# pashtari/factorizer

Measured on AMD Instinct MI355X. Metric: volumes/sec fwd+bwd, Swin Factorizer 128^3, higher is better.
Workload: dtype f32

## Files before the change

### factorizer_amd/csrc/nmf_cf.h

```cpp
#pragma once
#include <cstdlib>

#include "fz_common.h"
#include "nmf_core.h"
#include "nmf_gram.h"

namespace fz {

struct CfGeom {
  int B, C, D, H, W;
  int h;
  int G0, G1, G2;
  int s0, s1, s2;
  int accumulate;
  int divisor;
  float gscale_div;
  int64_t plane;
  int ps0, ps1, ps2;
};

enum { CF_PLAIN = 0, CF_STORE_FACTORS = 1, CF_FROM_FACTORS = 2 };
constexpr int CFG_COFAC = 88;

struct CfWave {
  using F = float;
  int lane;
  __device__ __forceinline__ int col(int j) const {
    const int jp = j >> 2, e = j & 3;
    return (((jp * 4 + (lane >> 4)) * 8 + ((lane >> 1) & 7)) * 8) + (lane & 1) * 4 + e;
  }
  __device__ __forceinline__ float sum(float v) const { return wave_sum(v); }
  __device__ __forceinline__ void sum8(float (&v)[8]) const { wave_sum8(v, lane); }
  __device__ __forceinline__ void st_priv(float* base, int idx, float v) const { base[idx * 64 + lane] = v; }
  __device__ __forceinline__ float ld_priv(const float* base, int idx) const { return base[idx * 64 + lane]; }
  __device__ __forceinline__ void st_uni(float* base, int idx, float v) const {
    if (lane == 0) base[idx] = v;
  }
  __device__ __forceinline__ float ld_uni(const float* base, int idx) const { return base[idx]; }
  __device__ __forceinline__ float ld_uni_global(const float* p, int idx) const { return p[idx]; }
  __device__ __forceinline__ float ld_v0(const float* v0, int j, int r, int R) const { return v0[col(j) * R + r]; }
  __device__ __forceinline__ float keep_col(int, float v) const { return v; }
  __device__ __forceinline__ void fence() const { __builtin_amdgcn_fence(__ATOMIC_ACQ_REL, "wavefront"); }
  static constexpr bool kDistRows = true;
  __device__ __forceinline__ float sum8_dist(const float (&v)[8]) const { return wave_sum8_dist(v, lane); }
  __device__ __forceinline__ float grp_take(float d, int m) const {
    return __int_as_float(__builtin_amdgcn_readlane(__float_as_int(d), 8 * m));
  }
  __device__ __forceinline__ bool grp_below(int n) const { return (lane >> 3) < n; }
  __device__ __forceinline__ void st_grp(float* base, int i0, int stride, float d) const {
    if ((lane & 7) == 0) base[i0 + (lane >> 3) * stride] = d;
  }
  __device__ __forceinline__ float ld_grp_global(const float* p, int i0, int stride) const { return p[i0 + (lane >> 3) * stride]; }
  __device__ __forceinline__ float ld_grp(const float* base, int i0, int stride) const { return base[i0 + (lane >> 3) * stride]; }
  __device__ __forceinline__ float grp_sum(float d) const { return wave_group_sum(d); }
  __device__ __forceinline__ float mask_rows(float d, int mreal) const { return (lane >> 3) < mreal ? d : 0.f; }
  __device__ __forceinline__ float pick_call(int c, float tot, float mine) const { return (lane & 7) == c ? tot : mine; }
  __device__ __forceinline__ void k_unrotate(float* scratch, float mine, float (&Kd)[8]) const {
    const int g = lane >> 3;
    scratch[g * 8 + ((g + lane) & 7)] = mine;
    fence();
    const float4 a = *reinterpret_cast<const float4*>(scratch + g * 8), b = *reinterpret_cast<const float4*>(scratch + g * 8 + 4);
    Kd[0] = a.x; Kd[1] = a.y; Kd[2] = a.z; Kd[3] = a.w; Kd[4] = b.x; Kd[5] = b.y; Kd[6] = b.z; Kd[7] = b.w;
    fence();
  }
};

struct CfAddr {
  int64_t base;
  int64_t off[2];
  int64_t V;
};

__device__ __forceinline__ void cf_decode(const CfGeom& q, int64_t mat, int lane, CfAddr& a) {
  unsigned t = (unsigned)mat;
  const int g2 = (int)(t % (unsigned)q.G2); t /= (unsigned)q.G2;
  const int g1 = (int)(t % (unsigned)q.G1); t /= (unsigned)q.G1;
  const int g0 = (int)(t % (unsigned)q.G0); t /= (unsigned)q.G0;
  const int hh = (int)(t % (unsigned)q.h);
  const int b = (int)(t / (unsigned)q.h);
  const int p1 = (lane >> 1) & 7, half = lane & 1;
  int z1 = g1 * 8 + p1 - q.s1; if (z1 < 0) z1 += q.H;
  int z2 = g2 * 8 + half * 4 - q.s2; if (z2 < 0) z2 += q.W;
  a.V = q.plane;
  a.base = ((int64_t)b * q.C + (int64_t)hh * 8) * a.V;
#pragma unroll
  for (int jp = 0; jp < 2; ++jp) {
    int z0 = g0 * 8 + jp * 4 + (lane >> 4) - q.s0; if (z0 < 0) z0 += q.D;
    a.off[jp] = ((int64_t)z0 * q.H + z1) * q.W + z2;
  }
}

template <typename AT>
__device__ __forceinline__ void cf_load(const AT* __restrict__ t, const CfAddr& a, float (&x)[8][8]) {
#pragma unroll
  for (int dd = 0; dd < 8; ++dd)
#pragma unroll
    for (int jp = 0; jp < 2; ++jp) {
      const float4 v = ld4(t + a.base + dd * a.V + a.off[jp]);
      x[dd][jp * 4 + 0] = v.x; x[dd][jp * 4 + 1] = v.y; x[dd][jp * 4 + 2] = v.z; x[dd][jp * 4 + 3] = v.w;
    }
}

__device__ __forceinline__ bool cf_pow2(float dv) { return (__float_as_uint(dv) & 0x007fffffu) == 0u && dv > 0.f; }

__device__ __forceinline__ void cf_divide(float (&g)[8][8], float dv) {
  if (dv == 1.0f) return;
  if (cf_pow2(dv)) {
    const float inv = 1.0f / dv;
#pragma unroll
    for (int dd = 0; dd < 8; ++dd)
#pragma unroll
      for (int j = 0; j < 8; ++j) g[dd][j] = g[dd][j] * inv;
  } else {
#pragma unroll
    for (int dd = 0; dd < 8; ++dd)
#pragma unroll
      for (int j = 0; j < 8; ++j) g[dd][j] = g[dd][j] / dv;
  }
}

__device__ __forceinline__ float4 cf_divide4(float4 o, float dv, bool pow2) {
  if (pow2) {
    const float inv = 1.0f / dv;
    o.x *= inv; o.y *= inv; o.z *= inv; o.w *= inv;
  } else {
    o.x /= dv; o.y /= dv; o.z /= dv; o.w /= dv;
  }
  return o;
}

__device__ __forceinline__ int64_t cf_logical_block(int xcd_remap) {
  const int64_t nb = gridDim.x;
  const int64_t bid = (xcd_remap & 2) ? nb - 1 - (int64_t)blockIdx.x : (int64_t)blockIdx.x;
  if (!(xcd_remap & 1) || nb < 16) return bid;
  const int64_t q = nb / 8, r = nb % 8, xcd = bid % 8, i = bid / 8;
  return (xcd < r ? xcd * (q + 1) : r * (q + 1) + (xcd - r) * q) + i;
}

template <int WPB>
struct CfTile {
  static constexpr bool SWZ = WPB == 8 || WPB == 4;
  static constexpr int LW = SWZ ? WPB * 8 : WPB * 8 + 8;
  static constexpr int NT = WPB * 64;
  static constexpr int CHUNKS = WPB * 2;
  static constexpr int STAGE_FLOATS = 2 * 64 * LW;
  static __device__ __forceinline__ int at(int row, int chunk) {
    if (WPB == 8) return row * LW + ((chunk ^ (2 * (row & 7))) << 2);
    if (WPB == 4) return row * LW + ((chunk ^ (2 * (((row >> 1) & 1) | ((((row & 1) ^ (row >> 2)) & 1) << 1)))) << 2);
    return row * LW + chunk * 4;
  }
};

template <typename AT>
__device__ __forceinline__ const AT* cf_at(const AT* p, unsigned o) {
  return reinterpret_cast<const AT*>(reinterpret_cast<const char*>(p) + o * (unsigned)sizeof(AT));
}
template <typename AT>
__device__ __forceinline__ AT* cf_at(AT* p, unsigned o) {
  return reinterpret_cast<AT*>(reinterpret_cast<char*>(p) + o * (unsigned)sizeof(AT));
}
template <bool HALF, typename AT>
__device__ __forceinline__ float4 cf_ld4(const AT* p, unsigned o, unsigned o2) {
  if (HALF) {
    float a[2], b[2];
    aload<2>(cf_at(p, o), a);
    aload<2>(cf_at(p, o2), b);
    return make_float4(a[0], a[1], b[0], b[1]);
  }
  return ld4(cf_at(p, o));
}
template <bool HALF, typename AT>
__device__ __forceinline__ void cf_st4(AT* p, unsigned o, unsigned o2, float4 v) {
  if (HALF) {
    const float a[2] = {v.x, v.y}, b[2] = {v.z, v.w};
    astore<2>(cf_at(p, o), a);
// ... 121 lines not shown
```

### factorizer_amd/csrc/nmf_cf.hip

```cpp
#include "nmf_cf.h"

namespace fz {

static void cf_norm_shift(const int* shift, int D, int H, int W, int (&s)[3]) {
  const int S[3] = {D, H, W};
  for (int i = 0; i < 3; ++i) { s[i] = shift[i] % S[i]; if (s[i] < 0) s[i] += S[i]; }
}

static int cf_geom(CfGeom& q, int B, int C, int D, int H, int W, const int* shift, const int* prev_shift, int accumulate,
                   int divisor) {
  if (B < 0 || C < 8 || (C % 8) || D < 8 || H < 8 || W < 8 || (D % 8) || (H % 8) || (W % 8))
    return fail(FZ_E_SHAPE, "fz_nmf_cf: needs C % 8 == 0 and spatial dims multiples of 8");
  if (!shift) return fail(FZ_E_ARG, "fz_nmf_cf: shift is null");
  if ((int64_t)D * H * W >= ((int64_t)1 << 30)) return fail(FZ_E_UNSUPPORTED, "fz_nmf_cf: 2^30 or more voxels per channel plane");
  q.B = B; q.C = C; q.D = D; q.H = H; q.W = W; q.h = C / 8; q.G0 = D / 8; q.G1 = H / 8; q.G2 = W / 8;
  int s[3], ps[3] = {0, 0, 0};
  cf_norm_shift(shift, D, H, W, s);
  if (s[2] % 2) return fail(FZ_E_UNSUPPORTED, "fz_nmf_cf: W-axis shift must be even");
  if (prev_shift) cf_norm_shift(prev_shift, D, H, W, ps);
  q.s0 = s[0]; q.s1 = s[1]; q.s2 = s[2];
  q.ps0 = ps[0]; q.ps1 = ps[1]; q.ps2 = ps[2];
  q.accumulate = accumulate; q.divisor = divisor; q.gscale_div = 1.0f;
  q.plane = (int64_t)D * H * W;
#ifdef FZ_PROBE_PLANE_PAD
  q.plane += FZ_PROBE_PLANE_PAD;
#endif
  return FZ_OK;
}

template <class Checks>
static int cf_prepare(CfLaunch& a, int B, int C, int D, int H, int W, const int* shift, const int* prev_shift, int accumulate,
                      int divisor, fz_stream_t stream, Checks checks) {
  int rc = cf_geom(a.q, B, C, D, H, W, shift, prev_shift, accumulate, divisor);
  if (rc == FZ_OK) rc = checks(a.q);
  if (rc != FZ_OK) return rc;
  a.nmat = (int64_t)B * a.q.h * a.q.G0 * a.q.G1 * a.q.G2;
  if (a.nmat >= (int64_t)1 << 31) return fail(FZ_E_UNSUPPORTED, "fz_nmf_cf: more than 2^31 matrices");
  a.xr = 1 | (tile_order() << 1);
  a.st = (hipStream_t)stream;
  return FZ_OK;
}

template <class F>
static int cf_with_dtype(int act_dtype, const char* bad, F f) {
  if (act_dtype == FZ_STORE_F32) return f(float{});
  if (act_dtype == FZ_STORE_BF16) return f(bf16{});
  return fail(FZ_E_ARG, bad);
}

}

using namespace fz;

extern "C" int fz_nmf_cf_supported(int C, int D, int H, int W, int d, int pd, int ph, int pw, int R, int T, int Tgrad) {
  if (d != 8 || pd != 8 || ph != 8 || pw != 8 || (C % 8) || (D % 8) || (H % 8) || (W % 8)) return 0;
  if (R < 1 || R > 2 || T < 0 || (int64_t)D * H * W >= ((int64_t)1 << 30)) return 0;
  const int G = Tgrad < 0 ? 0 : (Tgrad > T ? T : Tgrad);
  const int per_wave = (R == 1 ? Hist<8, 8, 1>::floats(G) : Hist<8, 8, 2>::floats(G)) * (int)sizeof(float);
  return per_wave <= 160 * 1024 ? 1 : 0;
}

extern "C" int fz_nmf_cf_fwd(const void* t, const float* u0, const float* v0, void* out, int B, int C, int D,
                             int H, int W, const int* shift, int accumulate, int divisor, int R, int T,
                             int solver, float eps, int act_dtype, fz_stream_t stream) {
  return cf_with_dtype(act_dtype, "fz_nmf_cf_fwd: bad act_dtype", [&](auto at) {
    using AT = decltype(at);
    CfLaunch a;
    const int rc = cf_prepare(a, B, C, D, H, W, shift, nullptr, accumulate, divisor, stream, [&](const CfGeom&) {
      if (!t || !u0 || !v0 || !out) return fail(FZ_E_ARG, "fz_nmf_cf_fwd: null pointer");
      if (R < 1 || R > 2) return fail(FZ_E_UNSUPPORTED, "fz_nmf_cf_fwd: rank 1..2");
      if (solver < FZ_SOLVER_MU || solver > FZ_SOLVER_SMU) return fail(FZ_E_ARG, "fz_nmf_cf_fwd: bad solver");
      return (int)FZ_OK;
    });
    if (rc != FZ_OK || a.nmat == 0) return rc;
    return cf_fwd_launch<AT>((const AT*)t, u0, v0, (AT*)out, nullptr, nullptr, a, CF_PLAIN, R, T, solver, eps);
  });
}

extern "C" int fz_nmf_cf_bwd(const void* t, const float* u0, const float* v0, const void* ga, void* gt, int B,
                             int C, int D, int H, int W, const int* shift, int accumulate, int nshift,
                             int relu_gate, int R, int T, int Tgrad, int solver, float eps, int act_dtype,
                             fz_stream_t stream) {
  return cf_with_dtype(act_dtype, "fz_nmf_cf_bwd: bad act_dtype", [&](auto at) {
    using AT = decltype(at);
    CfLaunch a;
    const int rc = cf_prepare(a, B, C, D, H, W, shift, nullptr, accumulate, 1, stream, [&](const CfGeom&) {
      if (!t || !u0 || !v0 || !ga || !gt) return fail(FZ_E_ARG, "fz_nmf_cf_bwd: null pointer");
      if (R < 1 || R > 2) return fail(FZ_E_UNSUPPORTED, "fz_nmf_cf_bwd: rank 1..2");
      if (solver < FZ_SOLVER_MU || solver > FZ_SOLVER_SMU) return fail(FZ_E_ARG, "fz_nmf_cf_bwd: bad solver");
      return (int)FZ_OK;
    });
    if (rc != FZ_OK || a.nmat == 0) return rc;
    a.q.gscale_div = (float)(nshift > 1 ? nshift : 1);
    const int G = Tgrad < 0 ? 0 : (Tgrad > T ? T : Tgrad);
    return cf_bwd_launch<AT>((const AT*)t, u0, v0, (const AT*)ga, (AT*)gt, a, relu_gate, R, T, G, solver, eps);
  });
}

extern "C" int fz_nmf_cf_factors_supported(int C, int D, int H, int W, int d, int pd, int ph, int pw, int R, int T, int Tgrad,
                                           int nshift, const int* shifts) {
  if (!fz_nmf_cf_supported(C, D, H, W, d, pd, ph, pw, R, T, Tgrad)) return 0;
  if (R != 1 || nshift != 2 || !shifts || (W % 64)) return 0;
  for (int w = 0; w < 2; ++w) {
    int s[3];
    cf_norm_shift(shifts + 3 * w, D, H, W, s);
    if (s[2] % 4) return 0;
  }
  return 1;
}

static int cf_fwd_factors(const void* t, const float* u0, const float* v0, void* out, float* vfac, float* ufac, int B, int C,
                          int D, int H, int W, const int* shift, const int* prev_shift, int form, int divisor, int R, int T,
                          int solver, float eps, int act_dtype, fz_stream_t stream, const char* null_msg, const char* dtype_msg) {
  return cf_with_dtype(act_dtype, dtype_msg, [&](auto at) {
    using AT = decltype(at);
    CfLaunch a;
    const int rc = cf_prepare(a, B, C, D, H, W, shift, prev_shift, form == CF_FROM_FACTORS, divisor, stream, [&](const CfGeom& q) {
      if (!t || !u0 || !v0 || !vfac || !ufac || (form == CF_FROM_FACTORS && (!out || !prev_shift))) return fail(FZ_E_ARG, null_msg);
      if (R != 1) return fail(FZ_E_UNSUPPORTED, "fz_nmf_cf_fwd factor forms: rank 1 only");
      if (W % 64) return fail(FZ_E_UNSUPPORTED, "fz_nmf_cf_fwd factor forms: W must be a multiple of 64");
      if (solver < FZ_SOLVER_MU || solver > FZ_SOLVER_SMU) return fail(FZ_E_ARG, "fz_nmf_cf_fwd factor forms: bad solver");
      if (divisor < 1) return fail(FZ_E_ARG, "fz_nmf_cf_fwd factor forms: divisor < 1");
      if ((q.s2 % 4) || (q.ps2 % 4)) return fail(FZ_E_UNSUPPORTED, "fz_nmf_cf_fwd factor forms: W-axis shift must be a multiple of 4");
      return (int)FZ_OK;
    });
    if (rc != FZ_OK || a.nmat == 0) return rc;
    return cf_fwd_launch<AT>((const AT*)t, u0, v0, (AT*)out, vfac, ufac, a, form, R, T, solver, eps);
  });
}

extern "C" int fz_nmf_cf_fwd_store_factors(const void* t, const float* u0, const float* v0, float* vfac, float* ufac, int B,
                                           int C, int D, int H, int W, const int* shift, int R, int T, int solver, float eps,
                                           int act_dtype, fz_stream_t stream) {
  return cf_fwd_factors(t, u0, v0, nullptr, vfac, ufac, B, C, D, H, W, shift, nullptr, CF_STORE_FACTORS, 1, R, T, solver, eps,
                        act_dtype, stream, "fz_nmf_cf_fwd_store_factors: null pointer (t, u0, v0, vfac or ufac)",
                        "fz_nmf_cf_fwd_store_factors: bad act_dtype");
}

extern "C" int fz_nmf_cf_fwd_from_factors(const void* t, const float* u0, const float* v0, const float* vfac,
                                          const float* ufac, void* out, int B, int C, int D, int H, int W, const int* shift,
                                          const int* prev_shift, int divisor, int R, int T, int solver, float eps, int act_dtype,
                                          fz_stream_t stream) {
  return cf_fwd_factors(t, u0, v0, out, const_cast<float*>(vfac), const_cast<float*>(ufac), B, C, D, H, W, shift, prev_shift,
                        CF_FROM_FACTORS, divisor, R, T, solver, eps, act_dtype, stream,
                        "fz_nmf_cf_fwd_from_factors: null pointer (t, u0, v0, vfac, ufac, out or prev_shift)",
                        "fz_nmf_cf_fwd_from_factors: bad act_dtype");
}

extern "C" int fz_nmf_cf_bwd_factors_supported(int C, int D, int H, int W, int d, int pd, int ph, int pw, int R, int T, int Tgrad,
                                               int solver, int relu_gate, int nshift, const int* shifts) {
  if (FZ_KNOB("FZ_CF_BWD_FACTORS").set && FZ_KNOB("FZ_CF_BWD_FACTORS").val == 0) return 0;
  if (!fz_nmf_cf_factors_supported(C, D, H, W, d, pd, ph, pw, R, T, Tgrad, nshift, shifts)) return 0;
  if (solver != FZ_SOLVER_HALS || !relu_gate) return 0;
  if (T < 1 || Tgrad < T) return 0;
  if ((C / 8) * (int64_t)(D / 8) * (H / 8) * (W / 8) >= ((int64_t)1 << 31)) return 0;
  const int lds = (CfTile<4>::STAGE_FLOATS + 4 * gram_hist_floats(T - 1) + 4 * 8 * CFG_COFAC) * (int)sizeof(float);
  return lds <= 64 * 1024 ? 1 : 0;
}

static int cf_bwd_factors(const void* t, const float* v0, const void* ga, void* gt, float* gcfac, float* cofac, int B, int C,
                          int D, int H, int W, const int* shift, const int* prev_shift, int form, int nshift, int T, int Tgrad,
                          float eps, int act_dtype, fz_stream_t stream, const char* null_msg, const char* dtype_msg) {
  return cf_with_dtype(act_dtype, dtype_msg, [&](auto at) {
    using AT = decltype(at);
    CfLaunch a;
    int rc = cf_prepare(a, B, C, D, H, W, shift, prev_shift, form == CF_FROM_FACTORS, 1, stream, [&](const CfGeom& q) {
      if (!t || !v0 || !ga || !gcfac || !cofac || (form == CF_FROM_FACTORS && (!gt || !prev_shift))) return fail(FZ_E_ARG, null_msg);
      if (W % 64) return fail(FZ_E_UNSUPPORTED, "fz_nmf_cf_bwd factor forms: W must be a multiple of 64");
      if (nshift != 2) return fail(FZ_E_UNSUPPORTED, "fz_nmf_cf_bwd factor forms: exactly two windows");
      if (T < 1 || Tgrad < T) return fail(FZ_E_UNSUPPORTED, "fz_nmf_cf_bwd factor forms: every iteration graded (1 <= T <= Tgrad)");
      if ((q.s2 % 4) || (q.ps2 % 4)) return fail(FZ_E_UNSUPPORTED, "fz_nmf_cf_bwd factor forms: W-axis shift must be a multiple of 4");
      return (int)FZ_OK;
    });
    if (rc != FZ_OK || a.nmat == 0) return rc;
    a.q.gscale_div = (float)nshift;
    rc = cf_bwd_gram_factors_launch<AT>((const AT*)t, v0, (const AT*)ga, (AT*)gt, gcfac, cofac, a, form, T, T, eps);
    if (rc == FZ_E_UNSUPPORTED) return fail(rc, "fz_nmf_cf_bwd factor forms: history exceeds the LDS budget");
    return rc;
  });
}

extern "C" int fz_nmf_cf_bwd_store_factors(const void* t, const float* v0, const void* ga, float* gcfac, float* cofac, int B,
                                           int C, int D, int H, int W, const int* shift, int nshift, int T, int Tgrad,
                                           float eps, int act_dtype, fz_stream_t stream) {
  return cf_bwd_factors(t, v0, ga, nullptr, gcfac, cofac, B, C, D, H, W, shift, nullptr, CF_STORE_FACTORS, nshift, T, Tgrad, eps,
                        act_dtype, stream, "fz_nmf_cf_bwd_store_factors: null pointer (t, v0, ga, gcfac or cofac)",
                        "fz_nmf_cf_bwd_store_factors: bad act_dtype");
}

extern "C" int fz_nmf_cf_bwd_from_factors(const void* t, const float* v0, const void* ga, const float* gcfac,
                                          const float* cofac, void* gt, int B, int C, int D, int H, int W, const int* shift,
                                          const int* prev_shift, int nshift, int T, int Tgrad, float eps, int act_dtype,
                                          fz_stream_t stream) {
  return cf_bwd_factors(t, v0, ga, gt, const_cast<float*>(gcfac), const_cast<float*>(cofac), B, C, D, H, W, shift, prev_shift,
                        CF_FROM_FACTORS, nshift, T, Tgrad, eps, act_dtype, stream,
                        "fz_nmf_cf_bwd_from_factors: null pointer (t, v0, ga, gcfac, cofac, gt or prev_shift)",
                        "fz_nmf_cf_bwd_from_factors: bad act_dtype");
}
```

### factorizer_amd/csrc/nmf_cf_gram.hip

```cpp
#include "nmf_cf.h"
#include "nmf_gram.h"

#ifndef FZ_GRAM_WAVES
#define FZ_GRAM_WAVES 3
#endif

namespace fz {

enum { CFG_HALVES = 0, CFG_RAW = 2 };

#ifdef FZ_PROBE_GRAM_NOMATH
#define FZ_GRAM_OUT_ROW(m, grow) probe_acc += grow[(m) & 7]
#else
#define FZ_GRAM_OUT_ROW(m, grow) P.out_row(m, grow)
#endif

template <typename AT> struct CfRaw;
template <> struct CfRaw<float> { using T = float4; };
template <> struct CfRaw<bf16> { using T = uint2; };

template <bool HALF>
__device__ __forceinline__ float4 cf_ld_raw(const float* p, unsigned o, unsigned o2) { return cf_ld4<HALF>(p, o, o2); }
template <bool HALF>
__device__ __forceinline__ uint2 cf_ld_raw(const bf16* p, unsigned o, unsigned o2) {
  if (HALF) {
    const unsigned a = *reinterpret_cast<const unsigned*>(cf_at(p, o)), b = *reinterpret_cast<const unsigned*>(cf_at(p, o2));
    return make_uint2(a, b);
  }
  return *reinterpret_cast<const uint2*>(cf_at(p, o));
}
__device__ __forceinline__ float4 cf_raw_f4(const float4& v) { return v; }
__device__ __forceinline__ float4 cf_raw_f4(const uint2& v) {
  return make_float4(__uint_as_float(v.x << 16), __uint_as_float(v.x & 0xffff0000u), __uint_as_float(v.y << 16),
                     __uint_as_float(v.y & 0xffff0000u));
}

template <typename AT>
__device__ __forceinline__ float cf_as_stored(float v) {
  if constexpr (sizeof(AT) == 2) {
    const f32v4 f = {v, v, v, v};
    const f32v4 r = __builtin_convertvector(__builtin_convertvector(f, bf16v4), f32v4);
    return r[0];
  }
  return v;
}

template <int WPB, bool HALF, typename AT, int MODE>
__global__ __launch_bounds__(WPB * 64, WPB == 4 ? FZ_GRAM_WAVES : 1) void nmf_cf_bwd_gram_kernel(
    const AT* __restrict__ t, const float* __restrict__ v0, const AT* __restrict__ ga, AT* __restrict__ gt, CfGeom q,
    int T, int G, float eps, int xcd_remap) {
  extern __shared__ __attribute__((aligned(16))) float fz_lds_cfg[];
  constexpr int FORM = CF_PLAIN;
  float* const gcfac = nullptr;
  float* const cofac = nullptr;
#include "nmf_cf_gram_body.inc"
}

template <typename AT, int MODE, int FORM>
__global__ __launch_bounds__(256, FZ_GRAM_WAVES) void nmf_cf_bwd_gram_fac_kernel(
    const AT* __restrict__ t, const float* __restrict__ v0, const AT* __restrict__ ga, AT* __restrict__ gt,
    float* __restrict__ gcfac, float* __restrict__ cofac, CfGeom q, int T, int G, float eps, int xcd_remap) {
  extern __shared__ __attribute__((aligned(16))) float fz_lds_cfg[];
  constexpr int WPB = 4;
  constexpr bool HALF = false;
#include "nmf_cf_gram_body.inc"
}

template <typename AT>
int cf_bwd_gram_launch(const AT* t, const float* v0, const AT* ga, AT* gt, const CfLaunch& a, int T, int G, float eps) {
  const CfGeom& q = a.q;
  const bool half = (q.s2 % 4) != 0;
#ifdef FZ_PROBE_GRAM_WPB
  const int twpb = (q.G2 % FZ_PROBE_GRAM_WPB) == 0 ? FZ_PROBE_GRAM_WPB : ((q.G2 % 4) == 0 ? 4 : 1);
#else
  const int twpb = (q.G2 % 4) == 0 ? 4 : 1;
#endif
  constexpr bool kF32 = sizeof(AT) == 4;
#ifdef FZ_PROBE_GRAM_WPB
  const int stage = twpb == FZ_PROBE_GRAM_WPB ? CfTile<FZ_PROBE_GRAM_WPB>::STAGE_FLOATS : (twpb == 4 ? CfTile<4>::STAGE_FLOATS : CfTile<1>::STAGE_FLOATS);
#else
  const int stage = twpb == 4 ? CfTile<4>::STAGE_FLOATS : CfTile<1>::STAGE_FLOATS;
#endif
  const int glds = (stage + twpb * gram_hist_floats(G - 1)) * (int)sizeof(float);
#ifndef FZ_PROBE_GRAM_WPB
  if (glds > 64 * 1024) return FZ_E_UNSUPPORTED;
#endif
  const unsigned nblk = (unsigned)(a.nmat / twpb);
#define FZ_CF_BWD_GRAM(WW, HH, MM) \
  hipLaunchKernelGGL((nmf_cf_bwd_gram_kernel<WW, HH, AT, MM>), dim3(nblk), dim3(64 * WW), glds, a.st, t, v0, ga, gt, q, T, G, eps, a.xr)
  constexpr int kRegMode = kF32 ? CFG_HALVES : CFG_RAW;
#ifdef FZ_PROBE_GRAM_WPB
  if (!half && twpb == FZ_PROBE_GRAM_WPB) {
    auto kern = nmf_cf_bwd_gram_kernel<FZ_PROBE_GRAM_WPB, false, AT, kRegMode>;
    if (glds > 64 * 1024) FZ_HIP_OK(hipFuncSetAttribute(reinterpret_cast<const void*>(kern), hipFuncAttributeMaxDynamicSharedMemorySize, glds));
    FZ_CF_BWD_GRAM(FZ_PROBE_GRAM_WPB, false, kRegMode);
    FZ_LAUNCH_CHECK();
    return FZ_OK;
  }
#endif
  if (half) { if (twpb == 4) FZ_CF_BWD_GRAM(4, true, kRegMode); else FZ_CF_BWD_GRAM(1, true, kRegMode); }
  else if (twpb == 4) FZ_CF_BWD_GRAM(4, false, kRegMode);
  else return FZ_E_UNSUPPORTED;
  FZ_LAUNCH_CHECK();
  return FZ_OK;
}
template <typename AT>
int cf_bwd_gram_factors_launch(const AT* t, const float* v0, const AT* ga, AT* gt, float* gcfac, float* cofac, const CfLaunch& a,
                               int form, int T, int G, float eps) {
  const CfGeom& q = a.q;
  if ((q.s2 % 4) || (q.ps2 % 4) || (q.G2 % 4) || G != T || G < 1) return FZ_E_UNSUPPORTED;
  int glds = (CfTile<4>::STAGE_FLOATS + 4 * gram_hist_floats(G - 1)) * (int)sizeof(float);
  if (form == CF_FROM_FACTORS) glds += 4 * 8 * CFG_COFAC * (int)sizeof(float);
  if (glds > 64 * 1024) return FZ_E_UNSUPPORTED;
  const unsigned nblk = (unsigned)(a.nmat / 4);
  constexpr int kRegMode = sizeof(AT) == 4 ? CFG_HALVES : CFG_RAW;
  if (form == CF_STORE_FACTORS)
    hipLaunchKernelGGL((nmf_cf_bwd_gram_fac_kernel<AT, kRegMode, CF_STORE_FACTORS>), dim3(nblk), dim3(256), glds, a.st, t, v0, ga,
                       gt, gcfac, cofac, q, T, G, eps, a.xr);
  else
    hipLaunchKernelGGL((nmf_cf_bwd_gram_fac_kernel<AT, kRegMode, CF_FROM_FACTORS>), dim3(nblk), dim3(256), glds, a.st, t, v0, ga,
                       gt, gcfac, cofac, q, T, G, eps, a.xr);
  FZ_LAUNCH_CHECK();
  return FZ_OK;
}
template int cf_bwd_gram_factors_launch<float>(const float*, const float*, const float*, float*, float*, float*, const CfLaunch&, int, int, int, float);
template int cf_bwd_gram_factors_launch<bf16>(const bf16*, const float*, const bf16*, bf16*, float*, float*, const CfLaunch&, int, int, int, float);

template int cf_bwd_gram_launch<float>(const float*, const float*, const float*, float*, const CfLaunch&, int, int, float);
template int cf_bwd_gram_launch<bf16>(const bf16*, const float*, const bf16*, bf16*, const CfLaunch&, int, int, float);

}
```

### factorizer_amd/csrc/nmf_cf_gram_body.inc

```
  static_assert(FORM == CF_PLAIN || (WPB == 4 && !HALF), "the factor forms: 4 patches per workgroup, W-axis shifts = 0 (mod 4)");
  using TL = CfTile<WPB>;
  using Raw = typename CfRaw<AT>::T;
  constexpr int NB = MODE == CFG_RAW ? 8 : 4;
  constexpr int IMG = 64 * TL::LW;
  float* S = fz_lds_cfg;
  const CfTileId id = cf_tile_id<WPB>(q, cf_logical_block(xcd_remap));
  const int tid = threadIdx.x, lane = tid & 63, wave = tid >> 6;
  int64_t base, V;
  unsigned off[2], off2[2];
  int lidx[2];
  cf_tile_decode<WPB>(q, id, tid, base, V, off, lidx, off2);
  const int own0 = cf_owner_lidx<WPB>(lane, wave, 0), own1 = cf_owner_lidx<WPB>(lane, wave, 1);
  float* hist = S + TL::STAGE_FLOATS + wave * gram_hist_floats(G - 1);

  float x[8][8];
#pragma unroll
  for (int dd = 0; dd < 8; ++dd)
#pragma unroll
    for (int k = 0; k < 2; ++k) {
      const float4 v = cf_ld4<HALF>(t + base + dd * V, off[k], off2[k]);
      x[dd][k * 4 + 0] = v.x; x[dd][k * 4 + 1] = v.y; x[dd][k * 4 + 2] = v.z; x[dd][k * 4 + 3] = v.w;
    }
  const int64_t bh = (int64_t)id.b * q.h + id.hh;
  const int64_t vol = (int64_t)q.D * q.H * q.W;
  const float* co[2];
  unsigned vcol[2];
  if constexpr (FORM == CF_FROM_FACTORS) {
    float* stage = S + TL::STAGE_FLOATS + WPB * gram_hist_floats(G - 1) + wave * (8 * CFG_COFAC);
    const int gp[3] = {id.g0, id.g1, id.gq * WPB + wave}, sh[3] = {q.s0, q.s1, q.s2}, ps[3] = {q.ps0, q.ps1, q.ps2};
    const int dim[3] = {q.D, q.H, q.W}, ng[3] = {q.G0, q.G1, q.G2};
    int o[3], pa[3][2];
#pragma unroll
    for (int a = 0; a < 3; ++a) {
      o[a] = gp[a] * 8 - sh[a] + ps[a];
      if (o[a] < 0) o[a] += dim[a];
      if (o[a] >= dim[a]) o[a] -= dim[a];
      pa[a][0] = o[a] >> 3;
      pa[a][1] = pa[a][0] + 1 == ng[a] ? 0 : pa[a][0] + 1;
    }
    const float* cp = cofac + bh * q.G0 * q.G1 * q.G2 * CFG_COFAC;
#pragma unroll
    for (int r = 0; r < 3; ++r) {
      const int i = lane + 64 * r, lp = i / (CFG_COFAC / 4), c4 = i % (CFG_COFAC / 4);
      if (i < 8 * (CFG_COFAC / 4)) {
        const int pidx = (pa[0][(lp >> 2) & 1] * q.G1 + pa[1][(lp >> 1) & 1]) * q.G2 + pa[2][lp & 1];
        *reinterpret_cast<float4*>(stage + lp * CFG_COFAC + c4 * 4) = ld4(cp + (int64_t)pidx * CFG_COFAC + c4 * 4);
      }
    }
    __builtin_amdgcn_fence(__ATOMIC_ACQ_REL, "wavefront");
    const int p12 = (lane >> 1) & 7, p2 = (lane & 1) * 4;
    int c1 = o[1] + p12; if (c1 >= q.H) c1 -= q.H;
    int c2 = o[2] + p2; if (c2 >= q.W) c2 -= q.W;
    const int b1 = (c1 >> 3) != pa[1][0], b2 = (c2 >> 3) != pa[2][0];
#pragma unroll
    for (int jp = 0; jp < 2; ++jp) {
      int c0 = o[0] + jp * 4 + (lane >> 4); if (c0 >= q.D) c0 -= q.D;
      const int b0 = (c0 >> 3) != pa[0][0];
      co[jp] = stage + (b0 * 4 + b1 * 2 + b2) * CFG_COFAC;
      vcol[jp] = (unsigned)((((c0 & 7) * 8 + (c1 & 7)) * 8) + (c2 & 7));
    }
  }
  cf_to_owner<WPB>(S, lidx, own0, own1, x);

  CfWave w{lane};
  GramBwd<8, CfWave> P;
  Raw gq[NB][2];
  auto request_g = [&]() {
#pragma unroll
    for (int dd = 0; dd < NB; ++dd)
#pragma unroll
      for (int k = 0; k < 2; ++k) gq[dd][k] = cf_ld_raw<HALF>(ga + base + dd * V, off[k], off2[k]);
  };
#ifdef FZ_PROBE_GRAM_NOMATH
  float probe_acc = 0.f;
  request_g();
#else
  P.forward(w, x, v0, 8, 512, T, G, eps, hist, request_g);
#endif
  asm volatile("" : "+s"(base));
#pragma unroll
  for (int bt = 0; bt < 8 / NB; ++bt) {
#pragma unroll
    for (int s = 0; s < NB / 2; ++s) {
#pragma unroll
      for (int c = 0; c < 2; ++c)
#pragma unroll
        for (int k = 0; k < 2; ++k) *reinterpret_cast<float4*>(S + c * IMG + lidx[k]) = cf_raw_f4(gq[2 * s + c][k]);
      if (MODE == CFG_HALVES && bt == 0 && s == NB / 2 - 1) {
#pragma unroll
        for (int dd = 0; dd < NB; ++dd)
#pragma unroll
          for (int k = 0; k < 2; ++k) gq[dd][k] = cf_ld_raw<HALF>(ga + base + (NB + dd) * V, off[k], off2[k]);
      }
      __syncthreads();
#pragma unroll
      for (int c = 0; c < 2; ++c) {
        const float4 a0 = *reinterpret_cast<const float4*>(S + c * IMG + own0);
        const float4 a1 = *reinterpret_cast<const float4*>(S + c * IMG + own1);
        const float grow[8] = {a0.x, a0.y, a0.z, a0.w, a1.x, a1.y, a1.z, a1.w};
        FZ_GRAM_OUT_ROW(NB * bt + 2 * s + c, grow);
      }
      __syncthreads();
    }
  }
  float4 gcq[2];
  auto request_gc0 = [&] {
    if constexpr (FORM == CF_FROM_FACTORS) {
#pragma unroll
      for (int k = 0; k < 2; ++k) gcq[k] = ld4(cf_at(gcfac + bh * vol, off[k]));
    }
  };
#ifdef FZ_PROBE_GRAM_NOMATH
  request_gc0();
#else
  P.reverse(w, x, 1.0f / q.gscale_div, request_gc0);
#endif
  if constexpr (FORM == CF_STORE_FACTORS) {
    *reinterpret_cast<float4*>(S + own0) = make_float4(P.gc[0], P.gc[1], P.gc[2], P.gc[3]);
    *reinterpret_cast<float4*>(S + own1) = make_float4(P.gc[4], P.gc[5], P.gc[6], P.gc[7]);
    __syncthreads();
    float* gp = gcfac + bh * vol;
#pragma unroll
    for (int k = 0; k < 2; ++k) st4(cf_at(gp, off[k]), *reinterpret_cast<const float4*>(S + lidx[k]));
    if ((lane & 7) == 0) {
      const int g = lane >> 3;
      float* cp = cofac + ((((bh * q.G0 + id.g0) * q.G1 + id.g1) * q.G2 + id.gq * WPB + wave) * CFG_COFAC);
      cp[g] = P.ud;
      cp[8 + g] = P.gsd;
      cp[16 + g] = P.ga1d;
      st4(cp + 24 + g * 8, make_float4(P.gKd[0], P.gKd[1], P.gKd[2], P.gKd[3]));
      st4(cp + 24 + g * 8 + 4, make_float4(P.gKd[4], P.gKd[5], P.gKd[6], P.gKd[7]));
    }
    return;
  }
  float gc0[8], vs0[8];
  if constexpr (FORM == CF_FROM_FACTORS) {
#pragma unroll
    for (int k = 0; k < 2; ++k) *reinterpret_cast<float4*>(S + lidx[k]) = gcq[k];
#pragma unroll
    for (int jp = 0; jp < 2; ++jp) {
#pragma unroll
      for (int e = 0; e < 4; ++e) vs0[jp * 4 + e] = v0[vcol[jp] + e];
    }
    __syncthreads();
    const float4 a0 = *reinterpret_cast<const float4*>(S + own0), a1 = *reinterpret_cast<const float4*>(S + own1);
    gc0[0] = a0.x; gc0[1] = a0.y; gc0[2] = a0.z; gc0[3] = a0.w; gc0[4] = a1.x; gc0[5] = a1.y; gc0[6] = a1.z; gc0[7] = a1.w;
    __syncthreads();
  }
#pragma unroll
  for (int bt = 0; bt < 8 / NB; ++bt) {
#pragma unroll
    for (int s = 0; s < NB / 2; ++s) {
      Raw old[2][2];
      if (FORM == CF_PLAIN && q.accumulate) {
#pragma unroll
        for (int c = 0; c < 2; ++c)
#pragma unroll
          for (int k = 0; k < 2; ++k) old[c][k] = cf_ld_raw<HALF>(gt + base + (NB * bt + 2 * s + c) * V, off[k], off2[k]);
      }
#pragma unroll
      for (int c = 0; c < 2; ++c) {
        const int m = NB * bt + 2 * s + c;
        float o[8];
#ifdef FZ_PROBE_GRAM_NOMATH
#pragma unroll
        for (int e = 0; e < 8; ++e) o[e] = x[m][e] + probe_acc;
#else
        float srow[8], gsm, ga1m;
        P.row_coeffs(w, m, srow, gsm, ga1m);
        P.gx_row(m, x, srow, gsm, ga1m, o);
#endif
#pragma unroll
        for (int e = 0; e < 8; ++e) o[e] = x[m][e] > 0.f ? o[e] : 0.f;
        if constexpr (FORM == CF_FROM_FACTORS) {
#pragma unroll
          for (int jp = 0; jp < 2; ++jp) {
            const float4 sa = *reinterpret_cast<const float4*>(co[jp] + 24 + m * 8);
            const float4 sb = *reinterpret_cast<const float4*>(co[jp] + 24 + m * 8 + 4);
            const float prow[8] = {sa.x, sa.y, sa.z, sa.w, sb.x, sb.y, sb.z, sb.w};
            const float pu = co[jp][m], pgs = co[jp][8 + m], pga1 = co[jp][16 + m];
#pragma unroll
            for (int e = 0; e < 4; ++e) {
              const int j = jp * 4 + e;
              const float g0 = gram_gx_elem<float, 8>(pu, gc0[j], pgs, pga1, vs0[j], prow, x, j);
              o[j] += cf_as_stored<AT>(x[m][j] > 0.f ? g0 : 0.f);
            }
          }
        }
        *reinterpret_cast<float4*>(S + c * IMG + own0) = make_float4(o[0], o[1], o[2], o[3]);
        *reinterpret_cast<float4*>(S + c * IMG + own1) = make_float4(o[4], o[5], o[6], o[7]);
      }
      __syncthreads();
#pragma unroll
      for (int c = 0; c < 2; ++c)
#pragma unroll
        for (int k = 0; k < 2; ++k) {
          float4 z = *reinterpret_cast<const float4*>(S + c * IMG + lidx[k]);
          if (FORM == CF_PLAIN && q.accumulate) {
            const float4 o = cf_raw_f4(old[c][k]);
            z.x += o.x; z.y += o.y; z.z += o.z; z.w += o.w;
          }
          cf_st4<HALF>(gt + base + (NB * bt + 2 * s + c) * V, off[k], off2[k], z);
        }
      __syncthreads();
    }
  }
```

### factorizer_amd/functional.py

```python
from __future__ import annotations

import ctypes
import math
import os

import torch

from . import _native as N


def _dev_guard(t: torch.Tensor):
    return torch.cuda.device(t.device)


class KernelTimer:

    def __init__(self, only=None):
        self.records = []
        self.only = None if only is None else set(only)

    def launch(self, name, nbytes, fn, cols=0, flops=0):
        if self.only is not None and name not in self.only:
            return fn()
        s = torch.cuda.Event(enable_timing=True)
# ... 195 lines not shown
        x, u0, v0 = ctx.saved_tensors
        T, G, solver, eps = ctx.cfg
        if G <= 0:
            return torch.zeros_like(x), None, None, None, None, None, None
        gx = _nmf_bwd_raw(x, u0, v0, gy.contiguous(), None, None, T, G, solver, eps)
        return gx, None, None, None, None, None, None


class NMFDecomposeFn(torch.autograd.Function):

    @staticmethod
    def forward(ctx, x, u0, v0, T, G, solver, eps):
        x = x.contiguous()
        u0 = u0.contiguous()
        v0 = v0.contiguous()
        _, u, v = _nmf_fwd_raw(x, u0, v0, T, solver, eps, want_uv=True)
        ctx.save_for_backward(x, u0, v0)
        ctx.cfg = (T, G, solver, eps)
        return u, v

    @staticmethod
    def backward(ctx, gu, gv):
        x, u0, v0 = ctx.saved_tensors
        T, G, solver, eps = ctx.cfg
        if G <= 0:
            return torch.zeros_like(x), None, None, None, None, None, None
        gx = _nmf_bwd_raw(x, u0, v0, None, gu.contiguous(), gv.contiguous(), T, G, solver, eps)
        return gx, None, None, None, None, None, None


def nmf(x, u0, v0, T, G, solver, eps=1e-16):
    return NMFFn.apply(x, u0, v0, T, G, solver, eps)


def nmf_decompose(x, u0, v0, T, G, solver, eps=1e-16):
    return NMFDecomposeFn.apply(x, u0, v0, T, G, solver, eps)


def gnmf_supported(M, N_, R, T, G) -> bool:
    return bool(N.lib().fz_gnmf_supported(int(M), int(N_), int(R), int(T), int(G)))


def _gnmf_ws(x, nmat, M, Nn, R, T, backward):
    nb = N.lib().fz_gnmf_workspace_bytes(nmat, M, Nn, R, T, int(backward))
    if nb < 0:
        raise N.NativeError("fz_gnmf_workspace_bytes failed")
    return torch.empty(max(nb // 4, 1), dtype=torch.float32, device=x.device)


def _gnmf_fwd_raw(x, u0, v0, T, solver, eps, want_uv=False):
    M, Nn = x.shape[-2:]
    R = u0.shape[1]
    nmat = x.numel() // (M * Nn)
    y = torch.empty_like(x)
    u = v = None
    if want_uv:
        u = torch.empty((*x.shape[:-2], M, R), dtype=x.dtype, device=x.device)
        v = torch.empty((*x.shape[:-2], Nn, R), dtype=x.dtype, device=x.device)
    ws = _gnmf_ws(x, nmat, M, Nn, R, T, False)
    with _dev_guard(x):
        rc = _timed(f"gnmf_fwd_{M}x{Nn}", 2 * x.numel() * 4, lambda: N.lib().fz_gnmf_fwd(
            x.data_ptr(), u0.data_ptr(), v0.data_ptr(), y.data_ptr(), N.ptr(u), N.ptr(v), nmat, M, Nn, R, T,
            N.SOLVER_ID[solver], eps, ws.data_ptr(), N.stream_ptr(x)))
    N.check(rc, "fz_gnmf_fwd")
    return y, u, v


def _gnmf_bwd_raw(x, u0, v0, gy, gu, gv, T, G, solver, eps):
    M, Nn = x.shape[-2:]
    R = u0.shape[1]
    nmat = x.numel() // (M * Nn)
    gx = torch.empty_like(x)
    ws = _gnmf_ws(x, nmat, M, Nn, R, T, True)
    with _dev_guard(x):
        rc = _timed(f"gnmf_bwd_{M}x{Nn}", 3 * x.numel() * 4, lambda: N.lib().fz_gnmf_bwd(
            x.data_ptr(), u0.data_ptr(), v0.data_ptr(), N.ptr(gy), N.ptr(gu), N.ptr(gv), gx.data_ptr(), nmat, M, Nn,
            R, T, G, N.SOLVER_ID[solver], eps, ws.data_ptr(), N.stream_ptr(x)))
    N.check(rc, "fz_gnmf_bwd")
    return gx


class GNMFFn(torch.autograd.Function):

    @staticmethod
    def forward(ctx, x, u0, v0, T, G, solver, eps):
        x, u0, v0 = x.contiguous(), u0.contiguous(), v0.contiguous()
        y, _, _ = _gnmf_fwd_raw(x, u0, v0, T, solver, eps)
        ctx.save_for_backward(x, u0, v0)
        ctx.cfg = (T, G, solver, eps)
        return y

    @staticmethod
    def backward(ctx, gy):
        x, u0, v0 = ctx.saved_tensors
        T, G, solver, eps = ctx.cfg
        if G <= 0:
            return torch.zeros_like(x), None, None, None, None, None, None
        return _gnmf_bwd_raw(x, u0, v0, gy.contiguous(), None, None, T, G, solver, eps), None, None, None, None, None, None


class GNMFDecomposeFn(torch.autograd.Function):
    @staticmethod
    def forward(ctx, x, u0, v0, T, G, solver, eps):
        x, u0, v0 = x.contiguous(), u0.contiguous(), v0.contiguous()
        _, u, v = _gnmf_fwd_raw(x, u0, v0, T, solver, eps, want_uv=True)
        ctx.save_for_backward(x, u0, v0)
        ctx.cfg = (T, G, solver, eps)
        return u, v

    @staticmethod
    def backward(ctx, gu, gv):
        x, u0, v0 = ctx.saved_tensors
        T, G, solver, eps = ctx.cfg
        if G <= 0:
            return torch.zeros_like(x), None, None, None, None, None, None
        gx = _gnmf_bwd_raw(x, u0, v0, None, gu.contiguous(), gv.contiguous(), T, G, solver, eps)
        return gx, None, None, None, None, None, None


def gnmf(x, u0, v0, T, G, solver, eps=1e-16):
    return GNMFFn.apply(x, u0, v0, T, G, solver, eps)


def gnmf_decompose(x, u0, v0, T, G, solver, eps=1e-16):
    return GNMFDecomposeFn.apply(x, u0, v0, T, G, solver, eps)


def nmf_cf_supported(geo: Geometry, R, T, G) -> bool:
    if len(geo.spatial) != 3 or any(s[2] % 2 for s in geo.shifts):
        return False
    return bool(N.lib().fz_nmf_cf_supported(geo.C, *geo.spatial, geo.d, *geo.patch, int(R), int(T), int(G)))


def nmf_cf_factors_supported(geo: Geometry, R, T, G) -> bool:
    if len(geo.spatial) != 3:
        return False
    k = (int(R), int(T), int(G))
    ok = geo._factors_ok.get(k)
    if ok is None:
        ok = geo._factors_ok[k] = bool(N.lib().fz_nmf_cf_factors_supported(geo.C, *geo.spatial, geo.d, *geo.patch, *k,
                                                                          geo.nshift, geo._carr))
    return ok


def nmf_cf_bwd_factors_supported(geo: Geometry, R, T, G, solver, relu_gate) -> bool:
    if len(geo.spatial) != 3:
        return False
    k = ("bwd", int(R), int(T), int(G), solver, bool(relu_gate))
    ok = geo._factors_ok.get(k)
    if ok is None:
        ok = geo._factors_ok[k] = bool(N.lib().fz_nmf_cf_bwd_factors_supported(
            geo.C, *geo.spatial, geo.d, *geo.patch, *k[1:4], N.SOLVER_ID[solver], int(k[5]), geo.nshift, geo._carr))
    return ok


def nmf_pcf_supported(geo: Geometry, R, T, G) -> bool:
    if os.environ.get("FZ_NMF_PCF", "1") == "0":
        return False
    return bool(N.lib().fz_nmf_pcf_supported(geo.C, *geo.s3, geo.d, *geo.p3, int(R), int(T), int(G)))


def nmf_core_supported(geo: Geometry, R, T, G) -> bool:
    return nmf_cf_supported(geo, R, T, G) or nmf_pcf_supported(geo, R, T, G)


def _core_launches(t, geo: Geometry, ad):
    lib, cols, tail = N.lib(), t.numel() // geo.C, (ad, N.stream_ptr(t))

    def launch(name, key, nbytes, *args):
        fn = getattr(lib, name)
        N.check(_timed(key, nbytes, cols=cols, fn=lambda: fn(*args, *tail)), name)

    return launch, f"{geo.C}x" + "x".join(str(v) for v in geo.spatial), [(N._i * 3)(*s) for s in geo.shifts3]


class FactCoreFn(torch.autograd.Function):

    @staticmethod
    def forward(ctx, t, u0, v0, geo, T, G, solver, eps, relu_gate):
        t = t.contiguous()
        u0, v0 = u0.contiguous(), v0.contiguous()
        B = t.shape[0]
        out = torch.empty_like(t)
        R = u0.shape[1]
        nt = t.element_size() * t.numel()
        hot = nmf_cf_supported(geo, R, T, G)
        launch, sp, shifts = _core_launches(t, geo, N.act_dtype(t))
        key = ("nmf_cf_fwd_" if hot else "nmf_pcf_fwd_") + sp
        lead = (t.data_ptr(), u0.data_ptr(), v0.data_ptr())
        dims = (B, geo.C, *geo.spatial) if hot else (B, geo.C, *geo.s3, *geo.p3)
        cfg = (R, T, N.SOLVER_ID[solver], eps)
        with _dev_guard(t):
            if hot and nmf_cf_factors_supported(geo, R, T, G):
                vfac = torch.empty((B, geo.h, *geo.spatial), device=t.device, dtype=torch.float32)
                ufac = torch.empty((B * geo.h * geo.G, 8), device=t.device, dtype=torch.float32)
                fac = (vfac.data_ptr(), ufac.data_ptr())
                nf = 4 * (t.numel() // 8)
                N.set_tile_order(0)
                launch("fz_nmf_cf_fwd_store_factors", key, nt + nf, *lead, *fac, *dims, shifts[0], *cfg)
                N.set_tile_order(1)
                launch("fz_nmf_cf_fwd_from_factors", key, 2 * nt + nf, *lead, *fac, out.data_ptr(), *dims, shifts[1], shifts[0], 2,
                       *cfg)
            else:
                name = "fz_nmf_cf_fwd" if hot else "fz_nmf_pcf_fwd"
                for w, arr in enumerate(shifts):
                    N.set_tile_order(w & 1)
                    launch(name, key, (3 if w else 2) * nt, *lead, out.data_ptr(), *dims, arr, int(w > 0),
                           geo.nshift if w == geo.nshift - 1 else 1, *cfg)
            N.set_tile_order(0)
        ctx.save_for_backward(t, u0, v0)
        ctx.cfg = (geo, T, G, solver, eps, relu_gate)
        return out

    @staticmethod
    def backward(ctx, ga):
        t, u0, v0 = ctx.saved_tensors
        geo, T, G, solver, eps, relu_gate = ctx.cfg
        if G <= 0:
            return (torch.zeros_like(t),) + (None,) * 8
        ga = ga.contiguous()
        if ga.dtype != t.dtype:
            ga = ga.to(t.dtype)
        gt = torch.empty_like(t)
        B = t.shape[0]
        R = u0.shape[1]
        nt = t.element_size() * t.numel()
        ad = N.act_dtype(t)
        hot = nmf_cf_supported(geo, R, T, G)
        launch, sp, shifts = _core_launches(t, geo, ad)
        key = ("nmf_cf_bwd_" if hot else "nmf_pcf_bwd_") + sp
        dims = (B, geo.C, *geo.spatial) if hot else (B, geo.C, *geo.s3, *geo.p3)
        with _dev_guard(t):
            if hot and nmf_cf_bwd_factors_supported(geo, R, T, G, solver, relu_gate):
                gcfac = torch.empty((B, geo.h, *geo.spatial), device=t.device, dtype=torch.float32)
                cofac = torch.empty((B * geo.h * geo.G, 88), device=t.device, dtype=torch.float32)
                lead = (t.data_ptr(), v0.data_ptr(), ga.data_ptr(), gcfac.data_ptr(), cofac.data_ptr())
                cfg = (geo.nshift, T, G, eps)
                nf = 4 * (t.numel() // 8) + 4 * cofac.numel()
                N.set_tile_order(0)
                launch("fz_nmf_cf_bwd_store_factors", key, 2 * nt + nf, *lead, *dims, shifts[0], *cfg)
                N.set_tile_order(1)
                launch("fz_nmf_cf_bwd_from_factors", key, 3 * nt + nf, *lead, gt.data_ptr(), *dims, shifts[1], shifts[0], *cfg)
            else:
                name = "fz_nmf_cf_bwd" if hot else "fz_nmf_pcf_bwd"
                lead = (t.data_ptr(), u0.data_ptr(), v0.data_ptr(), ga.data_ptr())
                cfg = (geo.nshift, int(relu_gate), R, T, G, N.SOLVER_ID[solver], eps)
                for w, arr in enumerate(shifts):
                    N.set_tile_order(w & 1)
                    if not hot and w > 0 and N.lib().fz_nmf_pcf_bwd_prefers_separate(*geo.p3, ad):
                        tmp = torch.empty_like(gt)
                        launch(name, key, 3 * nt, *lead, tmp.data_ptr(), *dims, arr, 0, *cfg)
                        launch("fz_act_add", "window_add_" + sp, 3 * nt, gt.data_ptr(), tmp.data_ptr(), gt.numel())
                        del tmp
                    else:
                        launch(name, key, (4 if w else 3) * nt, *lead, gt.data_ptr(), *dims, arr, int(w > 0), *cfg)
            N.set_tile_order(0)
        return (gt,) + (None,) * 8


def _k3(w):
    k = tuple(w.shape[4:])
    return (1,) * (3 - len(k)) + k


def _act_ok(*ts) -> bool:
    return ts[0].dtype in (torch.float32, torch.bfloat16) and all(t.dtype == ts[0].dtype for t in ts)


def gcorr_supported(inp, w) -> bool:
    if not (inp.is_cuda and inp.numel() and _act_ok(inp) and w.dtype == torch.float32):
        return False
    if inp.dim() not in (4, 5) or w.dim() != inp.dim() + 2 or w.shape[0] not in (1, inp.shape[0]):
        return False
    if not N.lib().fz_gcorr_supported(int(w.shape[3]), int(w.shape[2]), *_k3(w)):
        return False
    if torch.is_grad_enabled() and inp.requires_grad:
        return bool(N.lib().fz_gcorr_supported(int(w.shape[2]), int(w.shape[3]), *_k3(w)))
    return True


def _gcorr_raw(inp, w, add_eps=0.0, mul_a=None, mul_b=None):
    B = inp.shape[0]
    Bw, G, Co, Ci = w.shape[:4]
    sp = tuple(inp.shape[2:])
    D, H, W = (1,) * (3 - len(sp)) + sp
    if w.dtype != torch.float32 or not _act_ok(inp, *(t for t in (mul_a, mul_b) if t is not None)):
        raise TypeError("grouped correlation: activations of one type (float32 or bfloat16), float32 filters")
    out = torch.empty((B, G * Co, *sp), dtype=inp.dtype, device=inp.device)
    kd, kh, kw = _k3(w)
    with _dev_guard(inp):
        rc = _timed(f"gcorr_{Ci}->{Co}_k{kd}{kh}{kw}",
                    inp.element_size() * (inp.numel() + out.numel() * (3 if mul_a is not None else 1)),
                    lambda: N.lib().fz_gcorr_act(inp.data_ptr(), w.data_ptr(), out.data_ptr(), N.ptr(mul_a), N.ptr(mul_b), B, G,
                                                 Ci, Co, D, H, W, kd, kh, kw, int(Bw != 1), float(add_eps),
                                                 N.act_dtype(inp), N.stream_ptr(inp)))
    N.check(rc, "fz_gcorr_act")
    return out


def adjoint_filters(w):
    return torch.flip(w.transpose(2, 3), dims=tuple(range(4, w.ndim))).contiguous()


def _gcorr_wgrad_raw(inp, gout, w_shape):
    B = inp.shape[0]
    Bw, G, Co, Ci = w_shape[:4]
    sp = tuple(inp.shape[2:])
    D, H, W = (1,) * (3 - len(sp)) + sp
    ks = tuple(w_shape[4:])
    kd, kh, kw = (1,) * (3 - len(ks)) + ks
    if not _act_ok(inp, gout):
        raise TypeError("grouped correlation filter gradient: input and output gradient of one type (float32 or bfloat16)")
    gw = torch.empty(tuple(w_shape), dtype=torch.float32, device=inp.device)
    nb = N.lib().fz_gcorr_wgrad_workspace_bytes(B, G, Ci, Co, D, H, W, kd, kh, kw)
    ws = torch.empty(max(nb // 4, 1), dtype=torch.float32, device=inp.device)
    with _dev_guard(inp):
        rc = _timed(f"gcorr_wgrad_{Ci}->{Co}_k{kd}{kh}{kw}", inp.element_size() * (inp.numel() + gout.numel()),
                    lambda: N.lib().fz_gcorr_wgrad_act(inp.data_ptr(), gout.data_ptr(), gw.data_ptr(), ws.data_ptr(), B, G, Ci,
                                                       Co, D, H, W, kd, kh, kw, int(Bw != 1), N.act_dtype(inp),
                                                       N.stream_ptr(inp)))
    N.check(rc, "fz_gcorr_wgrad_act")
    return gw


def _gcorr_mu_bwd_raw(r, wT, g, s, num, eps, want):
    flags = [bool(f) for f in want]
    B = r.shape[0]
    Bw, G, Co, Ci = wT.shape[:4]
    sp = tuple(r.shape[2:])
    D, H, W = (1,) * (3 - len(sp)) + sp
    if wT.dtype != torch.float32 or not _act_ok(r, g, s, num):
        raise TypeError("multiplicative-update backward: activations of one type (float32 or bfloat16), float32 filters")
    outs = [torch.empty_like(s) if f else None for f in flags]
    kd, kh, kw = _k3(wT)
    with _dev_guard(r):
        rc = _timed(f"gcorr_mu_bwd_{Ci}->{Co}_k{kd}{kh}{kw}", r.element_size() * (r.numel() + s.numel() * (3 + sum(flags))),
                    lambda: N.lib().fz_gcorr_mu_bwd(r.data_ptr(), wT.data_ptr(), g.data_ptr(), s.data_ptr(), num.data_ptr(),
                                                    N.ptr(outs[0]), N.ptr(outs[1]), N.ptr(outs[2]), B, G, Ci, Co, D, H, W,
                                                    kd, kh, kw, int(Bw != 1), float(eps), N.act_dtype(r), N.stream_ptr(r)))
    N.check(rc, "fz_gcorr_mu_bwd")
    return outs


class GCorrFn(torch.autograd.Function):

    @staticmethod
    def forward(ctx, inp, w, add_eps):
        inp, w = inp.contiguous(), w.contiguous()
        ctx.save_for_backward(inp, w)
        return _gcorr_raw(inp, w, add_eps)

    @staticmethod
    def backward(ctx, gout):
        inp, w = ctx.saved_tensors
        gout = gout.contiguous()
        ginp = gw = None
        if ctx.needs_input_grad[0]:
            ginp = _gcorr_raw(gout, adjoint_filters(w))
        if ctx.needs_input_grad[1]:
            gw = _gcorr_wgrad_raw(inp, gout, w.shape)
        return ginp, gw, None


class GCorrMuFn(torch.autograd.Function):

    @staticmethod
    def forward(ctx, s, num, r, wT, eps):
        s, num, r, wT = s.contiguous(), num.contiguous(), r.contiguous(), wT.contiguous()
        ctx.save_for_backward(s, num, r, wT)
        ctx.eps = float(eps)
        return _gcorr_raw(r, wT, eps, s, num)

    @staticmethod
    def backward(ctx, g):
        s, num, r, wT = ctx.saved_tensors
        need = ctx.needs_input_grad
        ds, dnum, dden = _gcorr_mu_bwd_raw(r, wT, g.contiguous(), s, num, ctx.eps,
                                           (need[0], need[1], need[2] or need[3]))
        dr = _gcorr_raw(dden, adjoint_filters(wT)) if need[2] else None
        dwT = _gcorr_wgrad_raw(r, dden, wT.shape) if need[3] else None
        return ds, dnum, dr, dwT, None


class LagCorrFn(torch.autograd.Function):

    @staticmethod
    def forward(ctx, s, x, G, ksize):
        s, x = s.contiguous(), x.contiguous()
        ctx.save_for_backward(s, x)
        B = s.shape[0]
        return _gcorr_wgrad_raw(s, x, (B, G, x.shape[1] // G, s.shape[1] // G, *ksize))

    @staticmethod
    def backward(ctx, gL):
        s, x = ctx.saved_tensors
# ... 328 lines not shown
```

Baseline: 133.4.

## Share block-wide cofactor image across waves and reorder backward window launches

```diff
diff --git a/factorizer_amd/csrc/nmf_cf.h b/factorizer_amd/csrc/nmf_cf.h
--- a/factorizer_amd/csrc/nmf_cf.h
+++ b/factorizer_amd/csrc/nmf_cf.h
@@ -21,6 +21,7 @@
 
 enum { CF_PLAIN = 0, CF_STORE_FACTORS = 1, CF_FROM_FACTORS = 2 };
 constexpr int CFG_COFAC = 88;
+constexpr int CFG_COIMG = 20;
 
 struct CfWave {
   using F = float;
diff --git a/factorizer_amd/csrc/nmf_cf.hip b/factorizer_amd/csrc/nmf_cf.hip
--- a/factorizer_amd/csrc/nmf_cf.hip
+++ b/factorizer_amd/csrc/nmf_cf.hip
@@ -154,7 +154,7 @@
   if (solver != FZ_SOLVER_HALS || !relu_gate) return 0;
   if (T < 1 || Tgrad < T) return 0;
   if ((C / 8) * (int64_t)(D / 8) * (H / 8) * (W / 8) >= ((int64_t)1 << 31)) return 0;
-  const int lds = (CfTile<4>::STAGE_FLOATS + 4 * gram_hist_floats(T - 1) + 4 * 8 * CFG_COFAC) * (int)sizeof(float);
+  const int lds = (CfTile<4>::STAGE_FLOATS + 4 * gram_hist_floats(T - 1) + CFG_COIMG * CFG_COFAC) * (int)sizeof(float);
   return lds <= 64 * 1024 ? 1 : 0;
 }
 
diff --git a/factorizer_amd/csrc/nmf_cf_gram.hip b/factorizer_amd/csrc/nmf_cf_gram.hip
--- a/factorizer_amd/csrc/nmf_cf_gram.hip
+++ b/factorizer_amd/csrc/nmf_cf_gram.hip
@@ -110,7 +110,7 @@
   const CfGeom& q = a.q;
   if ((q.s2 % 4) || (q.ps2 % 4) || (q.G2 % 4) || G != T || G < 1) return FZ_E_UNSUPPORTED;
   int glds = (CfTile<4>::STAGE_FLOATS + 4 * gram_hist_floats(G - 1)) * (int)sizeof(float);
-  if (form == CF_FROM_FACTORS) glds += 4 * 8 * CFG_COFAC * (int)sizeof(float);
+  if (form == CF_FROM_FACTORS) glds += CFG_COIMG * CFG_COFAC * (int)sizeof(float);
   if (glds > 64 * 1024) return FZ_E_UNSUPPORTED;
   const unsigned nblk = (unsigned)(a.nmat / 4);
   constexpr int kRegMode = sizeof(AT) == 4 ? CFG_HALVES : CFG_RAW;
diff --git a/factorizer_amd/csrc/nmf_cf_gram_body.inc b/factorizer_amd/csrc/nmf_cf_gram_body.inc
--- a/factorizer_amd/csrc/nmf_cf_gram_body.inc
+++ b/factorizer_amd/csrc/nmf_cf_gram_body.inc
@@ -26,8 +26,8 @@
   const float* co[2];
   unsigned vcol[2];
   if constexpr (FORM == CF_FROM_FACTORS) {
-    float* stage = S + TL::STAGE_FLOATS + WPB * gram_hist_floats(G - 1) + wave * (8 * CFG_COFAC);
-    const int gp[3] = {id.g0, id.g1, id.gq * WPB + wave}, sh[3] = {q.s0, q.s1, q.s2}, ps[3] = {q.ps0, q.ps1, q.ps2};
+    float* image = S + TL::STAGE_FLOATS + WPB * gram_hist_floats(G - 1);
+    const int gp[3] = {id.g0, id.g1, id.gq * WPB}, sh[3] = {q.s0, q.s1, q.s2}, ps[3] = {q.ps0, q.ps1, q.ps2};
     const int dim[3] = {q.D, q.H, q.W}, ng[3] = {q.G0, q.G1, q.G2};
     int o[3], pa[3][2];
 #pragma unroll
@@ -40,23 +40,29 @@
     }
     const float* cp = cofac + bh * q.G0 * q.G1 * q.G2 * CFG_COFAC;
 #pragma unroll
-    for (int r = 0; r < 3; ++r) {
-      const int i = lane + 64 * r, lp = i / (CFG_COFAC / 4), c4 = i % (CFG_COFAC / 4);
-      if (i < 8 * (CFG_COFAC / 4)) {
-        const int pidx = (pa[0][(lp >> 2) & 1] * q.G1 + pa[1][(lp >> 1) & 1]) * q.G2 + pa[2][lp & 1];
-        *reinterpret_cast<float4*>(stage + lp * CFG_COFAC + c4 * 4) = ld4(cp + (int64_t)pidx * CFG_COFAC + c4 * 4);
-      }
-    }
-    __builtin_amdgcn_fence(__ATOMIC_ACQ_REL, "wavefront");
+    for (int r = 0; r < 2; ++r) {
+      const int i = tid + 256 * r, lp = i / (CFG_COFAC / 4), c4 = i % (CFG_COFAC / 4);
+      if (i < CFG_COIMG * (CFG_COFAC / 4)) {
+        const int dh = lp / 5;
+        int pw = pa[2][0] + lp % 5; if (pw >= q.G2) pw -= q.G2;
+#ifdef FZ_PROBE_CF_NOSTAGE
+        *reinterpret_cast<float4*>(image + lp * CFG_COFAC + c4 * 4) = make_float4(0.f, 0.f, 0.f, (float)(pw & dh));
+#else
+        const int pidx = (pa[0][dh >> 1] * q.G1 + pa[1][dh & 1]) * q.G2 + pw;
+        *reinterpret_cast<float4*>(image + lp * CFG_COFAC + c4 * 4) = ld4(cp + (int64_t)pidx * CFG_COFAC + c4 * 4);
+#endif
+      }
+    }
+    int o2 = o[2] + 8 * wave; if (o2 >= q.W) o2 -= q.W;
     const int p12 = (lane >> 1) & 7, p2 = (lane & 1) * 4;
     int c1 = o[1] + p12; if (c1 >= q.H) c1 -= q.H;
-    int c2 = o[2] + p2; if (c2 >= q.W) c2 -= q.W;
-    const int b1 = (c1 >> 3) != pa[1][0], b2 = (c2 >> 3) != pa[2][0];
+    int c2 = o2 + p2; if (c2 >= q.W) c2 -= q.W;
+    const int b1 = (c1 >> 3) != pa[1][0], b2 = (c2 >> 3) != (o2 >> 3);
 #pragma unroll
     for (int jp = 0; jp < 2; ++jp) {
       int c0 = o[0] + jp * 4 + (lane >> 4); if (c0 >= q.D) c0 -= q.D;
       const int b0 = (c0 >> 3) != pa[0][0];
-      co[jp] = stage + (b0 * 4 + b1 * 2 + b2) * CFG_COFAC;
+      co[jp] = image + ((b0 * 2 + b1) * 5 + wave + b2) * CFG_COFAC;
       vcol[jp] = (unsigned)((((c0 & 7) * 8 + (c1 & 7)) * 8) + (c2 & 7));
     }
   }
@@ -152,7 +158,12 @@
 #pragma unroll
     for (int s = 0; s < NB / 2; ++s) {
       Raw old[2][2];
-      if (FORM == CF_PLAIN && q.accumulate) {
+#ifdef FZ_PROBE_CF_PREREAD
+      constexpr bool kPreread = FORM == CF_FROM_FACTORS;
+#else
+      constexpr bool kPreread = false;
+#endif
+      if ((FORM == CF_PLAIN && q.accumulate) || kPreread) {
 #pragma unroll
         for (int c = 0; c < 2; ++c)
 #pragma unroll
@@ -196,7 +207,7 @@
 #pragma unroll
         for (int k = 0; k < 2; ++k) {
           float4 z = *reinterpret_cast<const float4*>(S + c * IMG + lidx[k]);
-          if (FORM == CF_PLAIN && q.accumulate) {
+          if ((FORM == CF_PLAIN && q.accumulate) || kPreread) {
             const float4 o = cf_raw_f4(old[c][k]);
             z.x += o.x; z.y += o.y; z.z += o.z; z.w += o.w;
           }
diff --git a/factorizer_amd/functional.py b/factorizer_amd/functional.py
--- a/factorizer_amd/functional.py
+++ b/factorizer_amd/functional.py
@@ -371,6 +371,14 @@
         ok = geo._factors_ok[k] = bool(N.lib().fz_nmf_cf_bwd_factors_supported(
             geo.C, *geo.spatial, geo.d, *geo.patch, *k[1:4], N.SOLVER_ID[solver], int(k[5]), geo.nshift, geo._carr))
     return ok
+
+
+def cf_bwd_factor_order(geo: Geometry, dtype):
+    if dtype == torch.float32:
+        aligned = [s[2] % 32 == 0 for s in geo.shifts3]
+        if aligned[0] and not aligned[1]:
+            return 1, 0
+    return 0, 1
 
 
 def nmf_pcf_supported(geo: Geometry, R, T, G) -> bool:
@@ -456,10 +464,12 @@
                 lead = (t.data_ptr(), v0.data_ptr(), ga.data_ptr(), gcfac.data_ptr(), cofac.data_ptr())
                 cfg = (geo.nshift, T, G, eps)
                 nf = 4 * (t.numel() // 8) + 4 * cofac.numel()
+                first, last = cf_bwd_factor_order(geo, t.dtype)
                 N.set_tile_order(0)
-                launch("fz_nmf_cf_bwd_store_factors", key, 2 * nt + nf, *lead, *dims, shifts[0], *cfg)
+                launch("fz_nmf_cf_bwd_store_factors", key, 2 * nt + nf, *lead, *dims, shifts[first], *cfg)
                 N.set_tile_order(1)
-                launch("fz_nmf_cf_bwd_from_factors", key, 3 * nt + nf, *lead, gt.data_ptr(), *dims, shifts[1], shifts[0], *cfg)
+                launch("fz_nmf_cf_bwd_from_factors", key, 3 * nt + nf, *lead, gt.data_ptr(), *dims, shifts[last], shifts[first],
+                       *cfg)
             else:
                 name = "fz_nmf_cf_bwd" if hot else "fz_nmf_pcf_bwd"
                 lead = (t.data_ptr(), u0.data_ptr(), v0.data_ptr(), ga.data_ptr())
```

New measurement: 134.5 (median of 6 runs). No clear change (+0.8%).
